# DeepMETv2/DeepMETv2

Hardware: AMD Instinct MI355X
Metric: events/sec (4.5k PF cands, k=16) (higher is better)
Workload: dtype f32

## Files before the change

### deepmetv2_amd/csrc/knn.hip

```cpp
#include <stdlib.h>

#include "common.h"
#include "nls_body.h"

namespace dmet {
namespace {

typedef float f2 __attribute__((ext_vector_type(2)));

constexpr int kTileC = 32;
constexpr int kQMax = 8;
constexpr int kMaxSplit = 8;
constexpr int kWavesPerGroup = 4;

__device__ __forceinline__ void wave_sync()
{
    __builtin_amdgcn_fence(__ATOMIC_RELEASE, "wavefront");
    __builtin_amdgcn_wave_barrier();
    __builtin_amdgcn_fence(__ATOMIC_ACQUIRE, "wavefront");
}

#define DMET_PKSUB_LO " op_sel:[0,0] op_sel_hi:[0,1] neg_lo:[0,1] neg_hi:[0,1]\n\t"
#define DMET_PKSUB_HI " op_sel:[1,0] op_sel_hi:[1,1] neg_lo:[0,1] neg_hi:[0,1]\n\t"
__device__ __forceinline__ void pk_dist_step4(f2 &accA, f2 &accB, f2 vxy, f2 vzw, f2 wxy, f2 wzw, f2 q0, f2 q1, f2 q2,
// ... 658 lines not shown
    const int64_t *ptr;
    int B;
    int64_t N;
    int k;
    float *nrm;
    uint8_t *rec;
    const KnnPlan *plan;
    const int32_t *order;
    const int32_t *pos_of;
    const int32_t *tile_ptr;
    float *psd;
    int32_t *psj;
    int32_t *nbr;
    float *dist;
    uint16_t *nbr16;
    int32_t *flags;
    int32_t *any;
    uint8_t *qflag;
    int32_t *qlist;
    const int32_t *xtile_ptr;
    int xtile_queries;
    int form2;
    float slack_scale;
    const float *rW, *rb;
    float *rP, *rQ;
    int r_sliced;
    int first_rider;
    int emit_coalesced;
    int no_rerank;
};

struct KnnSizeHint {
    int min_nodes = 0, max_nodes = 0;
};
thread_local KnnSizeHint g_size_hint;

struct KnnRider {
    const float *W = nullptr, *b = nullptr;
    float *P = nullptr, *Q = nullptr;
    int sliced = 0;
    bool done = false;
};
thread_local KnnRider g_rider;

struct KnnAffine {
    const float *raw = nullptr, *res = nullptr, *gamma = nullptr, *beta = nullptr, *mean = nullptr, *invstd = nullptr;
    bool done = false;
};
thread_local KnnAffine g_affine;
inline int rider_groups()
{
    static int cached = 0;
    if (cached == 0) {
        const char *e = getenv("DMET_KNN_RIDER_GROUPS");
        const int v = e ? atoi(e) : 0;
        cached = (v >= 1 && v <= 4096) ? v : 512;
    }
    return cached;
}

__device__ __forceinline__ void flag_query(const KnnFilterArgs &a, int q, int xtile)
{
    a.qflag[q] = 1;
    atomicAdd(a.flags + xtile, 1);
    const int slot = atomicAdd(a.any, 1);
    if (slot < a.N) a.qlist[slot] = q;
}

__device__ __forceinline__ unsigned bf16_rne_bits(float f)
{
    const unsigned u = __float_as_uint(f);
    return (u + 0x7fffu + ((u >> 16) & 1u)) >> 16;
}

constexpr int kRecFragBytes = 4 * kWave * 16;
constexpr int rec_bytes(int NH) { return kRecFragBytes * NH + 32 * 4; }
constexpr int kRecBytes = rec_bytes(1);
constexpr int kRecBytesMax = rec_bytes(2);

__device__ __forceinline__ int64_t rec_base_tile(const int64_t *__restrict__ ptr, int b) { return (ptr[b] >> 5) + b; }

constexpr int kRec16FragBytes = 2 * kWave * 16;
constexpr float kF16WideLimit = 16384.0f;

__device__ __forceinline__ bool f2_in_domain64(int64_t n) { return n >= kF2MinNodes && n <= kF2MaxNodes; }

template <int NH, bool AFFINE = false>
__global__ __launch_bounds__(256) void knn_prep_kernel(const float *__restrict__ x, const int64_t *__restrict__ ptr,
                                                        int B, int64_t N, float *__restrict__ nrm,
                                                        uint8_t *__restrict__ rec, int64_t nrec,
                                                        uint32_t *__restrict__ zero, size_t zero_bytes, KnnPlanOut o0,
                                                        KnnPlanOut o1, int form2, KnnAffine af = KnnAffine{})
{
    static_assert(!AFFINE || NH == 1, "the fused BatchNorm transform is built for 32 features");
    const int64_t t = (int64_t)blockIdx.x * blockDim.x + threadIdx.x;
    {
        const size_t words = zero_bytes >> 2, total = (size_t)gridDim.x * blockDim.x;
        for (size_t wd = (size_t)t; wd < words; wd += total) zero[wd] = 0u;
        if (t == 0)
            for (size_t bt = words << 2; bt < zero_bytes; ++bt) reinterpret_cast<uint8_t *>(zero)[bt] = 0;
    }
    if (blockIdx.x + 2 >= gridDim.x) {
        knn_plan_body(ptr, B, blockIdx.x + 2 == gridDim.x ? o0 : o1);
        return;
    }
    const int64_t tile = (int64_t)blockIdx.x * (blockDim.x >> 6) + __builtin_amdgcn_readfirstlane((int)(threadIdx.x >> 6));
    if (tile >= nrec) return;
    const int lane = (int)(t & 63), col = lane & 31, hh = lane >> 5;
    int lo = 0, hi = B;
    {
        const int ln = (int)(threadIdx.x & 63);
        while (hi - lo > 1) {
            const int span = hi - lo, step = (span + 63) >> 6;
            const int cand = lo + step * (ln + 1);
            const bool ok = cand < hi && rec_base_tile(ptr, cand) <= tile;
            const unsigned long long m = __ballot(ok);
            const int cnt = __popcll(m);
            const int nlo = lo + step * cnt;
            const int nhi = min(hi, lo + step * (cnt + 1));
            lo = __builtin_amdgcn_readfirstlane(nlo);
            hi = __builtin_amdgcn_readfirstlane(nhi);
        }
    }
    const int64_t ev_lo = ptr[lo], n = ptr[lo + 1] - ev_lo;
    const int64_t li0 = (tile - rec_base_tile(ptr, lo)) * 32;
    if (li0 >= n) return;
    const bool live = li0 + col < n;
    const int64_t r = ev_lo + (live ? li0 + col : 0);
    const bool rec16 = form2 != 0 && f2_in_domain64(n);
    float s = 0.0f;
    uint8_t *recp = rec + tile * rec_bytes(NH);
    float f[NH][16];
    if constexpr (NH == 1) {
        __shared__ __attribute__((aligned(16))) float prep_tile[4][32 * 36];
        float *T = prep_tile[threadIdx.x >> 6];
        const int fg = lane & 7;
        float4 mu4, sc4, be4;
        if constexpr (AFFINE) {
            mu4 = reinterpret_cast<const float4 *>(af.mean)[fg];
            const float4 is4 = reinterpret_cast<const float4 *>(af.invstd)[fg], ga4 = reinterpret_cast<const float4 *>(af.gamma)[fg];
            be4 = reinterpret_cast<const float4 *>(af.beta)[fg];
            sc4 = make_float4(ga4.x * is4.x, ga4.y * is4.y, ga4.z * is4.z, ga4.w * is4.w);
        }
#pragma unroll
        for (int jj = 0; jj < 4; ++jj) {
            const int rowj = 8 * jj + (lane >> 3);
            const bool livej = li0 + rowj < n;
            const int64_t rj = ev_lo + (livej ? li0 + rowj : 0);
            float4 v;
            if constexpr (AFFINE) {
                const float4 a = reinterpret_cast<const float4 *>(af.raw + rj * 32)[fg];
                v.x = (a.x - mu4.x) * sc4.x + be4.x; v.y = (a.y - mu4.y) * sc4.y + be4.y;
                v.z = (a.z - mu4.z) * sc4.z + be4.z; v.w = (a.w - mu4.w) * sc4.w + be4.w;
                if (af.res) {
                    const float4 q = reinterpret_cast<const float4 *>(af.res + rj * 32)[fg];
                    v.x += q.x; v.y += q.y; v.z += q.z; v.w += q.w;
                }
                if (livej) reinterpret_cast<float4 *>(const_cast<float *>(x) + rj * 32)[fg] = v;
            } else {
                v = reinterpret_cast<const float4 *>(x + rj * 32)[fg];
            }
            *reinterpret_cast<float4 *>(&T[rowj * 36 + 4 * fg]) = v;
        }
        asm volatile("s_waitcnt lgkmcnt(0)" ::: "memory");
        __builtin_amdgcn_wave_barrier();
#pragma unroll
        for (int kb = 0; kb < 2; ++kb) {
            const float4 v0 = *reinterpret_cast<const float4 *>(&T[col * 36 + 16 * kb + 8 * hh]);
            const float4 v1 = *reinterpret_cast<const float4 *>(&T[col * 36 + 16 * kb + 8 * hh + 4]);
            f[0][8 * kb + 0] = v0.x; f[0][8 * kb + 1] = v0.y; f[0][8 * kb + 2] = v0.z; f[0][8 * kb + 3] = v0.w;
            f[0][8 * kb + 4] = v1.x; f[0][8 * kb + 5] = v1.y; f[0][8 * kb + 6] = v1.z; f[0][8 * kb + 7] = v1.w;
        }
    } else {
#pragma unroll
        for (int half = 0; half < NH; ++half) {
#pragma unroll
            for (int kb = 0; kb < 2; ++kb) {
                const float4 *g = reinterpret_cast<const float4 *>(x + r * (32 * NH) + 32 * half + 16 * kb + 8 * hh);
                const float4 v0 = g[0], v1 = g[1];
                f[half][8 * kb + 0] = v0.x; f[half][8 * kb + 1] = v0.y; f[half][8 * kb + 2] = v0.z; f[half][8 * kb + 3] = v0.w;
                f[half][8 * kb + 4] = v1.x; f[half][8 * kb + 5] = v1.y; f[half][8 * kb + 6] = v1.z; f[half][8 * kb + 7] = v1.w;
            }
        }
    }
    bool wide = false;
#pragma unroll
    for (int half = 0; half < NH; ++half) {
#pragma unroll
        for (int u = 0; u < 16; ++u) {
            const float v = live ? f[half][u] : 0.0f;
            f[half][u] = v;
            s = __builtin_fmaf(v, v, s);
            wide = wide || !(__builtin_fabsf(v) < kF16WideLimit);
        }
    }
    s += __shfl_xor(s, 32, 64);
    if (rec16) {
        wide = wide || (__shfl_xor(wide ? 1 : 0, 32, 64) != 0);
#pragma unroll
        for (int half = 0; half < NH; ++half) {
            uint4 *dst = reinterpret_cast<uint4 *>(recp + half * kRec16FragBytes);
#pragma unroll
            for (int kb = 0; kb < 2; ++kb) {
                f16x8 hv;
#pragma unroll
                for (int u = 0; u < 8; ++u) hv[u] = wide ? (_Float16)0.0f : (_Float16)f[half][8 * kb + u];
                dst[kb * 64 + lane] = __builtin_bit_cast(uint4, hv);
            }
        }
        if (hh == 0) {
            reinterpret_cast<float *>(recp + kRec16FragBytes * NH)[col] =
                !live ? __builtin_inff() : (wide ? -__builtin_inff() : s);
            if (live) nrm[r] = s;
        }
        return;
    }
#pragma unroll
    for (int half = 0; half < NH; ++half) {
        unsigned h[16], m[16];
#pragma unroll
        for (int u = 0; u < 16; ++u) {
            const float v = f[half][u];
            h[u] = bf16_rne_bits(v);
            m[u] = bf16_rne_bits(v - __uint_as_float(h[u] << 16));
        }
        uint4 *dst = reinterpret_cast<uint4 *>(recp + half * kRecFragBytes);
#pragma unroll
        for (int kb = 0; kb < 2; ++kb) {
            dst[kb * 64 + lane] = make_uint4(h[8 * kb] | (h[8 * kb + 1] << 16), h[8 * kb + 2] | (h[8 * kb + 3] << 16),
                                             h[8 * kb + 4] | (h[8 * kb + 5] << 16), h[8 * kb + 6] | (h[8 * kb + 7] << 16));
            dst[(2 + kb) * 64 + lane] = make_uint4(m[8 * kb] | (m[8 * kb + 1] << 16), m[8 * kb + 2] | (m[8 * kb + 3] << 16),
                                                   m[8 * kb + 4] | (m[8 * kb + 5] << 16), m[8 * kb + 6] | (m[8 * kb + 7] << 16));
        }
    }
    if (!live) s = __builtin_inff();
    if (hh == 0) {
        reinterpret_cast<float *>(recp + kRecFragBytes * NH)[col] = s;
        if (live) nrm[r] = s;
    }
}

template <int NH = 1>
__device__ __forceinline__ f32x16 filter_block(const bf16x8 (&av)[4 * NH], const bf16x8 (&bv)[4 * NH], const f32x16 &cinit)
{
    f32x16 acc = cinit;
#pragma unroll
    for (int h = 0; h < NH; ++h) {
        acc = __builtin_amdgcn_mfma_f32_32x32x16_bf16(av[4 * h + 0], bv[4 * h + 0], acc, 0, 0, 0);
        acc = __builtin_amdgcn_mfma_f32_32x32x16_bf16(av[4 * h + 1], bv[4 * h + 1], acc, 0, 0, 0);
        acc = __builtin_amdgcn_mfma_f32_32x32x16_bf16(av[4 * h + 0], bv[4 * h + 2], acc, 0, 0, 0);
        acc = __builtin_amdgcn_mfma_f32_32x32x16_bf16(av[4 * h + 1], bv[4 * h + 3], acc, 0, 0, 0);
        acc = __builtin_amdgcn_mfma_f32_32x32x16_bf16(av[4 * h + 2], bv[4 * h + 0], acc, 0, 0, 0);
        acc = __builtin_amdgcn_mfma_f32_32x32x16_bf16(av[4 * h + 3], bv[4 * h + 1], acc, 0, 0, 0);
    }
    return acc;
}

template <int NH = 1>
__device__ __forceinline__ void filter_load(bf16x8 (&av)[4 * NH], f32x16 &cinit, const uint8_t *__restrict__ rec,
                                            int64_t tidx, int lane, int hh)
{
    const uint8_t *base = rec + tidx * rec_bytes(NH);
    const bf16x8 *g = reinterpret_cast<const bf16x8 *>(base);
#pragma unroll
    for (int m = 0; m < 4 * NH; ++m) av[m] = g[m * 64 + lane];
    const float4 *nr = reinterpret_cast<const float4 *>(base + kRecFragBytes * NH);
#pragma unroll
    for (int q = 0; q < 4; ++q) {
        const float4 v = nr[2 * q + hh];
        cinit[4 * q] = v.x; cinit[4 * q + 1] = v.y; cinit[4 * q + 2] = v.z; cinit[4 * q + 3] = v.w;
    }
}

template <int M>
struct FilterLane {
    float tk[M];
    float tau;
    int cnt;
    int kept;
    bool overflow;
};

constexpr int filter_list_len(int KP) { return KP + 4; }
constexpr int filter_queue_len(int M) { return M + 28; }

template <int QF>
struct FilterQueue {
    unsigned key[QF][kWave];
    unsigned short id[QF][kWave];
};

template <int M>
__device__ __forceinline__ void filter_drain(FilterLane<M> &L, FilterQueue<filter_queue_len(M)> &Q, int lane)
{
    constexpr int QF = filter_queue_len(M);
    int maxnew = L.cnt - L.kept;
#pragma unroll
// ... 263 lines not shown
                                (unsigned)local_id16(kj[p], ev_lo) | ((unsigned)local_id16(kj[p + 1], ev_lo) << 16);
                } else {
#pragma unroll
                    for (int p = 0; p < KP; ++p)
                        if (p < k) r16[p] = local_id16(kj[p], ev_lo);
                }
            }
            const float tau = L.tk[M - 1];
            const float nx = a.nrm[myq];
            const float an = __builtin_sqrtf(nx) * 1.000001f;
            const float rn = an + __builtin_sqrtf(fmaxf(kth, 0.0f)) * 1.00002f;
            const float slack = 2.0f * (4e-5f * an * rn + 1e-5f * rn * rn + 4e-6f * an * an) + 1e-30f;
            const bool full = tau < kKnnSentinel;
            if (L.overflow || !fits || (full && !(tau + nx - slack > kth))) {
                flag_query(a, myq, a.xtile_ptr[pos] + (myq - ev_lo) / a.xtile_queries);
            }
        }
        return;
    }
    if (a.no_rerank) {
        if (valid && sub == 0) flag_query(a, myq, a.xtile_ptr[pos] + (myq - ev_lo) / a.xtile_queries);
        return;
    }
    if (valid) {
        const int64_t slot = (int64_t)(tile - n_full) * kFQ + hh * 32 + col;
        float *ld = a.psd + (slot * nsub + sub) * MS;
        int32_t *lj = a.psj + (slot * nsub + sub) * MS;
        const float tfin = L.tk[M - 1];
        int out = 0;
        for (int pass = 0; pass < 2; ++pass)
            for (int s = 0; s < L.cnt; ++s) {
                const float key = __uint_as_float(Q.key[s][lane]);
                if ((pass == 0 ? key < tfin : key == tfin) && out < M) {
                    ld[out] = key;
                    lj[out] = ev_lo + (int32_t)Q.id[s][lane];
                    ++out;
                }
            }
        for (; out < M; ++out) { ld[out] = kKnnSentinel; lj[out] = -1; }
        ld[M] = L.tk[M - 1];
        lj[M] = (L.overflow || !fits) ? 1 : 0;
    }
}

template <int KP>
__global__ __launch_bounds__(kWave * kWavesPerGroup, 2) void knn_filter_kernel(const KnnFilterArgs a)
{
    __shared__ FilterQueue<filter_queue_len(filter_list_len(KP))> queue_all[kWavesPerGroup];
    const int wv = __builtin_amdgcn_readfirstlane(threadIdx.x >> 6), lane = threadIdx.x & 63;
    filter1_wave<KP>(a, queue_all[wv], (int)blockIdx.x, wv, lane);
}


#ifndef DMET_F2_DEFER
#define DMET_F2_DEFER 32
#endif
constexpr int kF2Defer = DMET_F2_DEFER;
#ifdef DMET_F2_LEAN
constexpr int kF2Slots = 26;
constexpr int kF2StageRows = 4;
constexpr int kF2WavesPerSimd = 3;
#else
constexpr int kF2Slots = 30;
constexpr int kF2StageRows = kWave;
constexpr int kF2WavesPerSimd = 2;
#endif
constexpr int kF2RowF = 16;
constexpr unsigned kF2TileBits = 11u, kF2TileMask = (1u << kF2TileBits) - 1u;

struct F2Wave {
    uint2 ent[kF2Slots][kWave];
    float rows[kF2StageRows][kF2RowF + 4];
};
#ifndef DMET_F2_LEAN
static_assert(sizeof(F2Wave) == 20480, "two workgroups of four wavefronts fill the CU's 160 KB exactly");
#else
static_assert(sizeof(F2Wave) * 12 <= 163840, "three workgroups of four wavefronts per CU");
#endif

template <int M>
struct F2Lane {
    float tk[M];
    float tau;
    int cnt;
    bool overflow;
};

template <int M>
__device__ __forceinline__ void f2_compact(F2Lane<M> &L, F2Wave &S, int lane, int limit)
{
    const float tauT = __uint_as_float(__float_as_uint(L.tau) & ~kF2TileMask);
    int maxcnt = L.cnt;
#pragma unroll
    for (int off = 32; off > 0; off >>= 1) maxcnt = max(maxcnt, __shfl_xor(maxcnt, off, 64));
    int out = 0;
    for (int s = 0; s < maxcnt; ++s) {
        if (s < L.cnt) {
            const uint2 e = S.ent[s][lane];
            if (!(__uint_as_float(e.y & ~kF2TileMask) > tauT)) { S.ent[out][lane] = e; ++out; }
        }
    }
    L.cnt = out;
    if (out > limit) {
        L.overflow = true;
        L.cnt = 0;
        L.tau = -__builtin_inff();
    }
}

template <int NH = 1>
struct F2Ops {
    f16x8 a[2 * NH];
    f32x16 c;
};

template <int NH = 1>
__device__ __forceinline__ f32x16 f2_block(const f16x8 (&av)[2 * NH], const f16x8 (&bv)[2 * NH], const f32x16 &cinit)
{
    f32x16 acc = cinit;
#pragma unroll
    for (int m = 0; m < 2 * NH; ++m) acc = __builtin_amdgcn_mfma_f32_32x32x16_f16(av[m], bv[m], acc, 0, 0, 0);
    return acc;
}

template <int NH = 1>
__device__ __forceinline__ void f2_load(F2Ops<NH> &o, const uint8_t *__restrict__ rec, int64_t tidx, int lane, int hh)
{
    const uint8_t *base = rec + tidx * rec_bytes(NH);
    const f16x8 *g = reinterpret_cast<const f16x8 *>(base);
#pragma unroll
    for (int m = 0; m < 2 * NH; ++m) o.a[m] = g[m * 64 + lane];
    const float4 *nr = reinterpret_cast<const float4 *>(base + kRec16FragBytes * NH);
#pragma unroll
    for (int q = 0; q < 4; ++q) {
        const float4 v = nr[2 * q + hh];
        o.c[4 * q] = v.x; o.c[4 * q + 1] = v.y; o.c[4 * q + 2] = v.z; o.c[4 * q + 3] = v.w;
    }
}

__device__ __forceinline__ float f2_slack(float an, float rn, float scale)
{
    return 2.0f * scale * (4e-5f * an * rn + 1e-5f * rn * rn + 4e-6f * an * an) + 1.96e-3f * an * rn + 6e-7f * (an + rn) +
           1e-30f;
}

constexpr int f2_list_len(int KP) { return KP <= 16 ? KP + 6 : KP + 4; }

__device__ __forceinline__ int f2_mask_row(int p) { return (p & 3) + 8 * ((p & 15) >> 2) + 4 * (p >> 4); }

template <int M, bool UPD, bool REC, bool INS, int NH = 1>
__device__ __forceinline__ void f2_tile(F2Lane<M> &L, F2Wave &S, const uint8_t *__restrict__ rec, int64_t rbase, int t,
                                        int t_hi, f32x16 &c0, f32x16 &c1, f32x16 &n0, f32x16 &n1, const F2Ops<NH> &use,
                                        F2Ops<NH> &ld, const f16x8 (&bq)[2][2 * NH], int lane, int hh, bool alive,
                                        float &carry)
{
#if defined(DMET_F2_ABL) && DMET_F2_ABL >= 2
    constexpr bool kRec = false;
#else
    constexpr bool kRec = REC;
#endif
#if defined(DMET_F2_ABL) && DMET_F2_ABL >= 3
    constexpr bool kUpd = false;
#else
    constexpr bool kUpd = UPD;
#endif
    if (kRec) {
        if (__any(L.cnt >= kF2Slots - 1)) f2_compact<M>(L, S, lane, kF2Slots - 3);
    }
#if defined(DMET_F2_SAMEREC)
    f2_load<NH>(ld, rec, rbase + (t & 1), lane, hh);
#else
    f2_load<NH>(ld, rec, rbase + min(t + 2, t_hi - 1), lane, hh);
#endif
    n0 = f2_block<NH>(use.a, bq[0], use.c);
    n1 = f2_block<NH>(use.a, bq[1], use.c);
    unsigned mask = 0u;
    if (kRec) {
        const auto tt = __builtin_amdgcn_permlane32_swap(__float_as_uint(L.tau), __float_as_uint(L.tau), false, false);
        const float t0 = __uint_as_float(tt[0]), t1 = __uint_as_float(tt[1]);
        unsigned ma = 0u, mb = 0u;
#pragma unroll
        for (int e = 0; e < 16; ++e) {
            ma = __builtin_amdgcn_alignbit(ma, __float_as_uint(c0[e] - t0), 31);
            mb = __builtin_amdgcn_alignbit(mb, __float_as_uint(c1[e] - t1), 31);
        }
        const auto mm = __builtin_amdgcn_permlane32_swap(ma, mb, false, false);
        mask = (mm[0] << 16) | mm[1];
    }
    float tmin = -__builtin_inff();
    if (kUpd) {
        float na = kKnnSentinel, nb = kKnnSentinel;
#pragma unroll
        for (int e = 0; e < 16; e += 2) {
            asm("v_min3_f32 %0, %0, %1, %2" : "+v"(na) : "v"(c0[e]), "v"(c0[e + 1]));
            asm("v_min3_f32 %0, %0, %1, %2" : "+v"(nb) : "v"(c1[e]), "v"(c1[e + 1]));
        }
        const auto nn = __builtin_amdgcn_permlane32_swap(__float_as_uint(na), __float_as_uint(nb), false, false);
        tmin = __uint_as_float(nn[0]);
        asm("v_min_f32 %0, %0, %1" : "+v"(tmin) : "v"(__uint_as_float(nn[1])));
    }
    if (kRec) {
        const unsigned packed = (__float_as_uint(tmin) & ~kF2TileMask) | (unsigned)t;
        S.ent[L.cnt][lane] = make_uint2(mask, packed);
        L.cnt += (mask != 0u) ? 1 : 0;
    }
    if (kUpd) {
        if (INS) {
            float v = tmin < -3.0e38f ? kKnnSentinel : tmin;
            asm("v_min_f32 %0, %0, %1" : "+v"(v) : "v"(carry));
            carry = kKnnSentinel;
#pragma unroll
            for (int p = M - 1; p >= 1; --p) L.tk[p] = __builtin_amdgcn_fmed3f(L.tk[p - 1], v, L.tk[p]);
            asm("v_min_f32 %0, %0, %1" : "+v"(L.tk[0]) : "v"(v));
            if (alive && !L.overflow) L.tau = L.tk[M - 1];
        } else {
            carry = tmin;
        }
    }
#ifdef DMET_F2_SCHED
#pragma unroll
    for (int g = 0; g < 12; ++g) {
        __builtin_amdgcn_sched_group_barrier(0x008, 1, 0);
        __builtin_amdgcn_sched_group_barrier(0x002, (kRec ? 11 : (kUpd ? 5 : 2)), 0);
    }
#endif
}

template <int M, bool UPD, bool REC, int NH = 1>
__device__ __forceinline__ void f2_sweep(F2Lane<M> &L, F2Wave &S, const uint8_t *__restrict__ rec, int64_t rbase,
                                         int t_lo, int t_hi, const f16x8 (&bq)[2][2 * NH], int lane, int hh, bool alive)
{
    if (t_lo >= t_hi) return;
    F2Ops<NH> A, B;
    f2_load<NH>(A, rec, rbase + t_lo, lane, hh);
    f32x16 c0 = f2_block<NH>(A.a, bq[0], A.c);
    f32x16 c1 = f2_block<NH>(A.a, bq[1], A.c);
    f32x16 n0, n1;
    f2_load<NH>(A, rec, rbase + min(t_lo + 1, t_hi - 1), lane, hh);
    float carry = kKnnSentinel;
    for (int t = t_lo; t < t_hi; t += 2) {
        f2_tile<M, UPD, REC, true, NH>(L, S, rec, rbase, t, t_hi, c0, c1, n0, n1, A, B, bq, lane, hh, alive, carry);
        if (t + 1 < t_hi)
            f2_tile<M, UPD, REC, true, NH>(L, S, rec, rbase, t + 1, t_hi, n0, n1, c0, c1, B, A, bq, lane, hh, alive, carry);
    }
}

__device__ __forceinline__ int filter_group(const KnnFilterArgs &a)
{
    const int full_groups = a.plan->n_full / kWavesPerGroup;
    return (int)blockIdx.x < full_groups ? xcd_swizzle((int)blockIdx.x, full_groups) : (int)blockIdx.x;
}

template <int KP, int NH = 1>
__device__ __forceinline__ void filter2_wave(const KnnFilterArgs &a, F2Wave &S, int *tickets, int group, int wv, int lane)
{
    constexpr int M = f2_list_len(KP);
    constexpr int D = 32 * NH;
    constexpr int MS = (M + 1 + 3) & ~3;
    const int col = lane & 31, hh = lane >> 5;
    const uint8_t *__restrict__ rec = a.rec;
    const int64_t *__restrict__ ptr = a.ptr;

    const int n_full = a.plan->n_full, split = a.plan->split, total = a.plan->total_tiles;
    const int item = group * kWavesPerGroup + wv;
    int tile = item, sub = 0, nsub = 1;
    if (item >= n_full) {
        const int r = item - n_full;
        tile = n_full + r / split;
        sub = r % split;
        nsub = split;
    }
    if (tile >= total) return;
    const int pos = find_tile_event(a.tile_ptr, a.B, tile);
    const int ev = a.order[pos];
    const int ev_lo = (int)ptr[ev], ev_hi = (int)ptr[ev + 1];
    const int q_first = ev_lo + (tile - a.tile_ptr[pos]) * kFQ;
    if (!f2_in_domain(ev_hi - ev_lo)) {
        if (NH != 1 && sub == 0) {
            const int q = q_first + lane;
            if (q < ev_hi) {
                flag_query(a, q, a.xtile_ptr[pos] + (q - ev_lo) / a.xtile_queries);
            }
        }
        return;
    }
    int clo = ev_lo, chi = ev_hi;
    bool idle_piece = false;
    if (nsub > 1) {
        if (ev_hi - ev_lo < kF2SplitMinNodes) {
            idle_piece = sub != 0;
        } else {
            const int chunk = (((chi - clo) + nsub - 1) / nsub + 31) & ~31;
            clo = min(chi, clo + sub * chunk);
            chi = min(chi, clo + chunk);
        }
    }
    const int64_t rbase = (ptr[ev] >> 5) + ev;
    const int64_t rlast = rbase + (ev_hi - ev_lo - 1) / 32;
    const int t_lo = (clo - ev_lo) / 32, t_hi = idle_piece ? t_lo : (chi - ev_lo + 31) / 32;

    const int myq = q_first + hh * 32 + col;
    const bool valid = myq < ev_hi;
    float t_fix = -__builtin_inff();
    bool act = valid;
    for (int attempt = 0;; ++attempt) {
    F2Lane<M> L;
#pragma unroll
    for (int p = 0; p < M; ++p) L.tk[p] = kKnnSentinel;
    L.tau = attempt == 0 ? -__builtin_inff() : t_fix;
    L.cnt = 0;
    L.overflow = false;
    {
        f16x8 bq[2][2 * NH];
#pragma unroll
        for (int b = 0; b < 2; ++b) {
            const int64_t qrec = min(rbase + (q_first - ev_lo) / 32 + b, rlast);
            const f16x8 *g = reinterpret_cast<const f16x8 *>(rec + qrec * rec_bytes(NH));
#pragma unroll
            for (int m = 0; m < 2 * NH; ++m) bq[b][m] = g[m * 64 + lane] * (_Float16)-2.0f;
        }
        if (attempt == 0) {
            const int t_def = min(t_hi, t_lo + kF2Defer);
            f2_sweep<M, true, false, NH>(L, S, rec, rbase, t_lo, t_def, bq, lane, hh, valid);
            f2_sweep<M, true, true, NH>(L, S, rec, rbase, t_def, t_hi, bq, lane, hh, valid);
            f2_sweep<M, false, true, NH>(L, S, rec, rbase, t_lo, t_def, bq, lane, hh, valid);
        } else {
            f2_sweep<M, false, true, NH>(L, S, rec, rbase, t_lo, t_hi, bq, lane, hh, valid);
        }
    }
    f2_compact<M>(L, S, lane, kF2Slots);
#if defined(DMET_F2_ABL) && DMET_F2_ABL >= 1
    return;
#endif

    const int64_t qrow_id = valid ? myq : ev_lo;
    float qrow[D];
    {
        const float4 *g = reinterpret_cast<const float4 *>(a.x + qrow_id * D);
#pragma unroll
        for (int c = 0; c < D / 4; ++c) {
            const float4 v = g[c];
            qrow[4 * c] = v.x; qrow[4 * c + 1] = v.y; qrow[4 * c + 2] = v.z; qrow[4 * c + 3] = v.w;
        }
    }
    unsigned long long kk[KP];
#pragma unroll
    for (int p = 0; p < KP; ++p) kk[p] = (unsigned long long)__float_as_uint(kKnnSentinel) << 32;
    const int nent = (act && !L.overflow) ? L.cnt : 0;
    int slot = 0;
    unsigned cmask = 0u;
    int ctile = 0;
    auto pop = [&]() __attribute__((always_inline)) -> int32_t {
        if (cmask == 0u && slot < nent) {
            const uint2 e = S.ent[slot][lane];
            cmask = e.x;
            ctile = (int)(e.y & kF2TileMask);
            ++slot;
        }
        int32_t j = -1;
        if (cmask != 0u) {
            const int r = __builtin_clz(cmask);
            cmask &= ~(0x80000000u >> r);
            j = ev_lo + ctile * 32 + f2_mask_row(r);
        }
        return j;
    };
    const float4 *x4 = reinterpret_cast<const float4 *>(a.x);
#ifdef DMET_RR_PRIO
    __builtin_amdgcn_s_setprio(DMET_RR_PRIO);
#endif
    if constexpr (NH != 1) {
        for (;;) {
            const int32_t j = pop();
            if (!__any(j >= 0)) break;
            const float4 *row = x4 + (int64_t)(j >= 0 ? j : ev_lo) * (D / 4);
            float4 v[D / 4];
#pragma unroll
            for (int c = 0; c < D / 4; ++c) v[c] = row[c];
            float dc = 0.0f;
#pragma unroll
            for (int c = 0; c < D / 4; ++c) {
                float df;
                df = v[c].x - qrow[4 * c + 0]; dc = __builtin_fmaf(df, df, dc);
                df = v[c].y - qrow[4 * c + 1]; dc = __builtin_fmaf(df, df, dc);
                df = v[c].z - qrow[4 * c + 2]; dc = __builtin_fmaf(df, df, dc);
                df = v[c].w - qrow[4 * c + 3]; dc = __builtin_fmaf(df, df, dc);
            }
            const unsigned long long nk =
                j >= 0 ? (((unsigned long long)__float_as_uint(dc) << 32) | (unsigned)j) : ~0ull;
            bool g[KP];
#pragma unroll
            for (int p = 0; p < KP; ++p) g[p] = kk[p] > nk;
// ... 153 lines not shown
                for (int t = 0; t < RP; ++t) {
                    const int pi = t * 64 + lane;
                    const uint4 v = *reinterpret_cast<const uint4 *>(stg + 4 * pi);
                    if ((on >> (pi / RP)) & 1ull) *reinterpret_cast<uint4 *>(a.nbr + blk + 4 * pi) = v;
                }
                wave_sync();
#pragma unroll
                for (int q = 0; q < RP; ++q)
                    *reinterpret_cast<uint4 *>(stg + lane * KP + 4 * q) =
                        make_uint4(__float_as_uint(kd[4 * q]), __float_as_uint(kd[4 * q + 1]), __float_as_uint(kd[4 * q + 2]),
                                   __float_as_uint(kd[4 * q + 3]));
                wave_sync();
#pragma unroll
                for (int t = 0; t < RP; ++t) {
                    const int pi = t * 64 + lane;
                    const uint4 v = *reinterpret_cast<const uint4 *>(stg + 4 * pi);
                    if ((on >> (pi / RP)) & 1ull) *reinterpret_cast<uint4 *>(a.dist + blk + 4 * pi) = v;
                }
                if (a.nbr16) {
                    if constexpr (KP % 8 == 0) {
                        constexpr int RH = KP / 8;
                        wave_sync();
#pragma unroll
                        for (int q = 0; q < RH; ++q) {
                            uint4 w;
                            w.x = (unsigned)local_id16(kj[8 * q], ev_lo) | ((unsigned)local_id16(kj[8 * q + 1], ev_lo) << 16);
                            w.y = (unsigned)local_id16(kj[8 * q + 2], ev_lo) | ((unsigned)local_id16(kj[8 * q + 3], ev_lo) << 16);
                            w.z = (unsigned)local_id16(kj[8 * q + 4], ev_lo) | ((unsigned)local_id16(kj[8 * q + 5], ev_lo) << 16);
                            w.w = (unsigned)local_id16(kj[8 * q + 6], ev_lo) | ((unsigned)local_id16(kj[8 * q + 7], ev_lo) << 16);
                            *reinterpret_cast<uint4 *>(stg + lane * (KP / 2) + 4 * q) = w;
                        }
                        wave_sync();
#pragma unroll
                        for (int t = 0; t < RH; ++t) {
                            const int pi = t * 64 + lane;
                            const uint4 v = *reinterpret_cast<const uint4 *>(stg + 4 * pi);
                            if ((on >> (pi / RH)) & 1ull)
                                *reinterpret_cast<uint4 *>(reinterpret_cast<unsigned *>(a.nbr16 + blk) + 4 * pi) = v;
                        }
                    } else if (rows_on) {
                        uint16_t *r16 = a.nbr16 + (int64_t)myq * k;
#pragma unroll
                        for (int p = 0; p + 1 < KP; p += 2)
                            reinterpret_cast<unsigned *>(r16)[p >> 1] =
                                (unsigned)local_id16(kj[p], ev_lo) | ((unsigned)local_id16(kj[p + 1], ev_lo) << 16);
                    }
                }
                wave_sync();
                return kth;
            }
        }
        if (!rows_on) return kth;
#pragma unroll
        for (int p = 0; p < KP; ++p) {
            if (p < k) {
                a.nbr[(int64_t)myq * k + p] = kj[p];
                a.dist[(int64_t)myq * k + p] = kd[p];
            }
        }
        if (a.nbr16) {
            uint16_t *r16 = a.nbr16 + (int64_t)myq * k;
            if ((k & 1) == 0) {
#pragma unroll
                for (int p = 0; p + 1 < KP; p += 2)
                    if (p < k)
                        reinterpret_cast<unsigned *>(r16)[p >> 1] =
                            (unsigned)local_id16(kj[p], ev_lo) | ((unsigned)local_id16(kj[p + 1], ev_lo) << 16);
            } else {
#pragma unroll
                for (int p = 0; p < KP; ++p)
                    if (p < k) r16[p] = local_id16(kj[p], ev_lo);
            }
        }
        return kth;
    };
    if (nsub == 1) {
        bool retry = false;
        const float kth = emit(act, true);
        if (act) {
            const float nx = a.nrm[myq];
            const float an = __builtin_sqrtf(nx) * 1.000001f;
            const float rn = an + __builtin_sqrtf(fmaxf(kth, 0.0f)) * 1.00002f;
            const float slack = f2_slack(an, rn, NH == 1 ? 1.0f : 1.5f);
            const bool full = tau < kKnnSentinel;
            const bool wideq = !(nx < kF16WideLimit * kF16WideLimit);
            const bool fail = L.overflow || wideq || (full && !(kth >= 0.0f && tau + nx - slack > kth));
            float ts = kth - nx + slack;
            ts += (__builtin_fabsf(ts) + nx + slack) * 4.8e-7f + 1e-30f;
            retry = fail && attempt == 0 && !L.overflow && !wideq && kth >= 0.0f && ts + nx - slack > kth &&
                    ts < kKnnSentinel;
            if (fail && !retry) {
                flag_query(a, myq, a.xtile_ptr[pos] + (myq - ev_lo) / a.xtile_queries);
#ifdef DMET_KNN_WHY
                a.qflag[myq] = (uint8_t)(1 | (L.overflow ? 2 : 0) | (wideq ? 4 : 0) | (kth < 0.0f ? 8 : 0) | (attempt ? 16 : 0) |
                                         (!(ts < kKnnSentinel) ? 32 : 0) | (!(ts + nx - slack > kth) ? 64 : 0));
                a.dist[(int64_t)myq * k + 0] = tau; a.dist[(int64_t)myq * k + 1] = kth; a.dist[(int64_t)myq * k + 2] = slack; a.dist[(int64_t)myq * k + 3] = (float)L.cnt;
#endif
            }
            t_fix = retry ? ts : -__builtin_inff();
        }
        if (!__any(retry)) return;
        act = retry;
        continue;
    }
    static_assert(kFilterMaxSplit == 2 && kWavesPerGroup % 2 == 0, "pairs of sub-sweeps share a workgroup");
    const int64_t fslot = (int64_t)(tile - n_full) * kFQ + hh * 32 + col;
    if (valid) {
        float *ld = a.psd + (fslot * nsub + sub) * MS;
        int32_t *lj = a.psj + (fslot * nsub + sub) * MS;
#pragma unroll
        for (int p = 0; p < KP; ++p) { ld[p] = kd[p]; lj[p] = kj[p]; }
        ld[M] = tau;
        lj[M] = L.overflow ? 1 : 0;
    }
    __builtin_amdgcn_fence(__ATOMIC_RELEASE, "workgroup");
    int arrived = 0;
    if (lane == 0) arrived = atomicAdd(&tickets[wv >> 1], 1);
    arrived = __builtin_amdgcn_readfirstlane(arrived);
    if (arrived == 0) return;
    __builtin_amdgcn_fence(__ATOMIC_ACQUIRE, "workgroup");
    float tau_o = kKnnSentinel;
    int of_o = 0;
    if (valid) {
        const float *ld = a.psd + (fslot * nsub + (sub ^ 1)) * MS;
        const int32_t *lj = a.psj + (fslot * nsub + (sub ^ 1)) * MS;
        tau_o = ld[M];
        of_o = lj[M];
#pragma unroll
        for (int p = 0; p < KP; ++p) {
            const float od = ld[p];
            const int32_t oj = lj[p];
            const unsigned long long nk = oj >= 0 ? (((unsigned long long)__float_as_uint(od) << 32) | (unsigned)oj) : ~0ull;
            bool g[KP];
#pragma unroll
            for (int q = 0; q < KP; ++q) g[q] = kk[q] > nk;
#pragma unroll
            for (int q = KP - 1; q >= 1; --q) kk[q] = g[q - 1] ? kk[q - 1] : (g[q] ? nk : kk[q]);
            kk[0] = g[0] ? nk : kk[0];
        }
#pragma unroll
        for (int p = 0; p < KP; ++p) {
            kd[p] = __uint_as_float((unsigned)(kk[p] >> 32));
            kj[p] = kd[p] == kKnnSentinel ? -1 : (int32_t)(unsigned)kk[p];
        }
        const float kth = emit(true, false);
        const float nx = a.nrm[myq];
        const float an = __builtin_sqrtf(nx) * 1.000001f;
        const float rn = an + __builtin_sqrtf(fmaxf(kth, 0.0f)) * 1.00002f;
        const float slack = f2_slack(an, rn, NH == 1 ? 1.0f : 1.5f);
        const bool wideq = !(nx < kF16WideLimit * kF16WideLimit);
        const bool fail_a = tau < kKnnSentinel && !(kth >= 0.0f && tau + nx - slack > kth);
        const bool fail_b = tau_o < kKnnSentinel && !(kth >= 0.0f && tau_o + nx - slack > kth);
        if (L.overflow || of_o != 0 || wideq || fail_a || fail_b)
            flag_query(a, myq, a.xtile_ptr[pos] + (myq - ev_lo) / a.xtile_queries);
    }
    return;
    }
}

template <int KP, int NH = 1>
__global__ __launch_bounds__(kWave * kWavesPerGroup, kF2WavesPerSimd) void knn_filter12_kernel(const KnnFilterArgs a)
{
    union WaveLds {
        F2Wave f2;
#ifndef DMET_F2_LEAN
        FilterQueue<filter_queue_len(filter_list_len(KP))> f1;
#endif
    };
    __shared__ WaveLds sh_all[kWavesPerGroup];
    if constexpr (NH == 1) {
        if (a.rP != nullptr && (int)blockIdx.x >= a.first_rider) {
            static_assert(sizeof(WaveLds) >= sizeof(float) * kNlsLdsFloats, "a wavefront's LDS holds the transposition tiles");
            const int rwv = __builtin_amdgcn_readfirstlane(threadIdx.x >> 6);
            const int64_t wave = (int64_t)((int)blockIdx.x - a.first_rider) * kWavesPerGroup + rwv;
            const int64_t nwaves = (int64_t)((int)gridDim.x - a.first_rider) * kWavesPerGroup;
            float *tp = reinterpret_cast<float *>(&sh_all[rwv]);
            if (a.r_sliced == 2)
                node_linear_split_bf16_wave<32, 32>(a.x, a.N, a.rW, a.rb, a.rP, reinterpret_cast<unsigned short *>(a.rQ), wave,
                                                    nwaves, threadIdx.x & 63);
            else if (a.r_sliced == 1) node_linear_split_wave<32, 32, true>(a.x, a.N, a.rW, a.rb, a.rP, a.rQ, tp, wave, nwaves, threadIdx.x & 63);
            else node_linear_split_wave<32, 32, false>(a.x, a.N, a.rW, a.rb, a.rP, a.rQ, tp, wave, nwaves, threadIdx.x & 63);
            return;
        }
    }
    static_assert(sizeof(WaveLds) == sizeof(F2Wave), "the union is sized by the second form");
#ifndef DMET_F2_LEAN
    static_assert(sizeof(FilterQueue<filter_queue_len(filter_list_len(KP))>) <= sizeof(F2Wave) - 8, "ticket bytes are free");
#endif
    static_assert(kWavesPerGroup / 2 <= 2, "two ticket words");
    int *tickets = reinterpret_cast<int *>(&sh_all[0].f2.rows[kF2StageRows - 1][kF2RowF + 2]);
    const int wv = __builtin_amdgcn_readfirstlane(threadIdx.x >> 6), lane = threadIdx.x & 63;
    if (threadIdx.x < kWavesPerGroup / 2) tickets[threadIdx.x] = 0;
    __syncthreads();
    const int group = filter_group(a);
    filter2_wave<KP, NH>(a, sh_all[wv].f2, tickets, group, wv, lane);
#ifndef DMET_F2_LEAN
    if constexpr (NH == 1) filter1_wave<KP>(a, sh_all[wv].f1, group, wv, lane);
#endif
}

template <int KP>
__global__ __launch_bounds__(256) void knn_rerank_kernel(const KnnFilterArgs a)
{
    constexpr int M = filter_list_len(KP);
    constexpr int MS = (M + 1 + 3) & ~3;
    constexpr int QPW = kWave / M;
    constexpr int QPB = 4 * QPW;
    constexpr int EMAX = kFilterMaxSplit * M;
    __shared__ float sc[QPB][EMAX];
    __shared__ int32_t sj[QPB][EMAX];
    __shared__ float skth[QPB];
    __shared__ int sfail[QPB];
    __shared__ float qbuf[QPB][32];
    constexpr int PARTS = (kFQ + QPB - 1) / QPB;
    const int wv = __builtin_amdgcn_readfirstlane(threadIdx.x >> 6), lane = threadIdx.x & 63;
    const int qw = lane / M, l = lane - qw * M;
    const int slot = wv * QPW + min(qw, QPW - 1);
    const int bid = blockIdx.x;
    if (a.form2 && a.plan->form1_events == 0) return;
    const int n_full = a.plan->n_full, split = a.plan->split;
    const int ft = n_full + bid / PARTS, part = bid % PARTS;
    if (ft >= a.plan->total_tiles) return;
    const int pos = find_tile_event(a.tile_ptr, a.B, ft);
    const int ev = a.order[pos];
    const int64_t ev_lo = a.ptr[ev], ev_hi = a.ptr[ev + 1];
    if (a.form2 && f2_in_domain((int)(ev_hi - ev_lo))) return;
    const int qoff = part * QPB + wv * QPW + qw;
    const int64_t q = ev_lo + (int64_t)(ft - a.tile_ptr[pos]) * kFQ + qoff;
    const bool active = qw < QPW && qoff < kFQ && q < ev_hi;
    const int64_t qq = active ? q : ev_lo;
    const int nsub = split;
    const int64_t fslot = (int64_t)(ft - n_full) * kFQ + (active ? qoff : 0);
    const float *bd = a.psd + fslot * nsub * MS;
    const int32_t *bj = a.psj + fslot * nsub * MS;
    const int E = nsub * M;
// ... 812 lines not shown
```

Baseline: 45890.

## Fold norm and threshold subtraction into an extra MFMA for the f16 KNN filter

For the 32-feature f16 filter path, the candidate norm is split into four f16 limbs stored in the record, and the running threshold tau is encoded as two f16 values. A leading MFMA then adds norm minus tau directly into the accumulator, so the per-element subtraction of tau before sign-bit mask extraction disappears. A conservative key lower bound and certification margins are added to keep the approximate tau exact-safe. The sweep is also reworked to triple-buffer records with a prefetch lead of three and to update the tau encoding only every other tile, trading an extra MFMA and more registers for fewer VALU ops.

```diff
diff --git a/deepmetv2_amd/csrc/knn.hip b/deepmetv2_amd/csrc/knn.hip
--- a/deepmetv2_amd/csrc/knn.hip
+++ b/deepmetv2_amd/csrc/knn.hip
@@ -764,6 +764,13 @@
 
 constexpr int kRec16FragBytes = 2 * kWave * 16;
 constexpr float kF16WideLimit = 16384.0f;
+static_assert(kRec16FragBytes + kWave * 16 <= rec_bytes(1) && 2 * kRec16FragBytes + kWave * 16 <= rec_bytes(2),
+              "the fold fragment fits the record");
+constexpr float kF2NormP[4] = {0x1p15f, 0x1p5f, 0x1p-6f, 0x1p-17f};
+constexpr float kF2NormInvP[4] = {0x1p-15f, 0x1p-5f, 0x1p6f, 0x1p17f};
+constexpr float kF2NormMax = 65504.0f * 0x1p15f;
+constexpr float kF2TauC[2] = {0x1p14f, 0x1p-15f};
+constexpr float kF2TauRepMax = 65504.0f * 0x1p14f;
 
 __device__ __forceinline__ bool f2_in_domain64(int64_t n) { return n >= kF2MinNodes && n <= kF2MaxNodes; }
 
@@ -890,11 +897,34 @@
                 dst[kb * 64 + lane] = __builtin_bit_cast(uint4, hv);
             }
         }
+        if constexpr (NH != 1) {
+            if (hh == 0) {
+                reinterpret_cast<float *>(recp + kRec16FragBytes * NH)[col] =
+                    !live ? __builtin_inff() : (wide ? -__builtin_inff() : s);
+                if (live) nrm[r] = s;
+            }
+            return;
+        }
+        f16x8 fv = {};
         if (hh == 0) {
-            reinterpret_cast<float *>(recp + kRec16FragBytes * NH)[col] =
-                !live ? __builtin_inff() : (wide ? -__builtin_inff() : s);
+            const float sn = !live ? __builtin_inff() : ((wide || !(s < kF2NormMax)) ? -__builtin_inff() : s);
+            if (sn == sn && __builtin_fabsf(sn) < __builtin_inff()) {
+                float rr = sn;
+#pragma unroll
+                for (int i = 0; i < 4; ++i) {
+                    const _Float16 h = (_Float16)(rr * kF2NormInvP[i]);
+                    fv[4 + i] = h;
+                    rr -= (float)h * kF2NormP[i];
+                }
+            } else {
+                fv[4] = (_Float16)sn;
+            }
             if (live) nrm[r] = s;
-        }
+        } else {
+            fv[0] = (_Float16)kF2TauC[0];
+            fv[1] = (_Float16)kF2TauC[1];
+        }
+        reinterpret_cast<uint4 *>(recp + kRec16FragBytes * NH)[lane] = __builtin_bit_cast(uint4, fv);
         return;
     }
 #pragma unroll
@@ -1324,6 +1354,8 @@
 struct F2Lane {
     float tk[M];
     float tau;
+    unsigned tq;
+    float rep;
     int cnt;
     bool overflow;
 };
@@ -1350,18 +1382,34 @@
     }
 }
 
+__device__ __forceinline__ f16x8 f2_fold(unsigned tq)
+{
+    const f16x8 pc = {(_Float16)0.0f, (_Float16)0.0f, (_Float16)0.0f, (_Float16)0.0f, (_Float16)kF2NormP[0],
+                      (_Float16)kF2NormP[1], (_Float16)kF2NormP[2], (_Float16)kF2NormP[3]};
+    uint4 u = __builtin_bit_cast(uint4, pc);
+    u.x = tq;
+    return __builtin_bit_cast(f16x8, u);
+}
+
 template <int NH = 1>
 struct F2Ops {
     f16x8 a[2 * NH];
+    f16x8 f;
+};
+template <>
+struct F2Ops<2> {
+    f16x8 a[4];
     f32x16 c;
 };
 
 template <int NH = 1>
-__device__ __forceinline__ f32x16 f2_block(const f16x8 (&av)[2 * NH], const f16x8 (&bv)[2 * NH], const f32x16 &cinit)
-{
-    f32x16 acc = cinit;
-#pragma unroll
-    for (int m = 0; m < 2 * NH; ++m) acc = __builtin_amdgcn_mfma_f32_32x32x16_f16(av[m], bv[m], acc, 0, 0, 0);
+__device__ __forceinline__ f32x16 f2_block(const F2Ops<NH> &o, const f16x8 (&bv)[2 * NH], unsigned tq)
+{
+    f32x16 acc;
+    if constexpr (NH == 1) acc = __builtin_amdgcn_mfma_f32_32x32x16_f16(o.f, f2_fold(tq), f32x16{}, 0, 0, 0);
+    else acc = o.c;
+#pragma unroll
+    for (int m = 0; m < 2 * NH; ++m) acc = __builtin_amdgcn_mfma_f32_32x32x16_f16(o.a[m], bv[m], acc, 0, 0, 0);
     return acc;
 }
 
@@ -1372,29 +1420,61 @@
     const f16x8 *g = reinterpret_cast<const f16x8 *>(base);
 #pragma unroll
     for (int m = 0; m < 2 * NH; ++m) o.a[m] = g[m * 64 + lane];
-    const float4 *nr = reinterpret_cast<const float4 *>(base + kRec16FragBytes * NH);
-#pragma unroll
-    for (int q = 0; q < 4; ++q) {
-        const float4 v = nr[2 * q + hh];
-        o.c[4 * q] = v.x; o.c[4 * q + 1] = v.y; o.c[4 * q + 2] = v.z; o.c[4 * q + 3] = v.w;
-    }
-}
+    if constexpr (NH == 1) {
+        o.f = g[2 * NH * 64 + lane];
+    } else {
+        const float4 *nr = reinterpret_cast<const float4 *>(base + kRec16FragBytes * NH);
+#pragma unroll
+        for (int q = 0; q < 4; ++q) {
+            const float4 v = nr[2 * q + hh];
+            o.c[4 * q] = v.x; o.c[4 * q + 1] = v.y; o.c[4 * q + 2] = v.z; o.c[4 * q + 3] = v.w;
+        }
+    }
+}
+
+__device__ __forceinline__ unsigned f2_tau16(float tau, float &rep)
+{
+    const float x = __builtin_amdgcn_fmed3f(-tau * (1.0f / kF2TauC[0]), -65504.0f, 65504.0f);
+    float v = __builtin_amdgcn_fmed3f(__builtin_fmaf(__builtin_fabsf(x), -0x1p-9f, x), -65504.0f, 65504.0f);
+    const float y0 = (float)__builtin_amdgcn_cvt_pkrtz(v, v)[0];
+    const float w = __builtin_fmaf(-y0, kF2TauC[0] / kF2TauC[1], x * (kF2TauC[0] / kF2TauC[1]));
+    v = fminf(__builtin_fmaf(__builtin_fabsf(w), -0x1p-9f, w - 0x1p-24f), 65504.0f);
+    const auto y = __builtin_amdgcn_cvt_pkrtz(y0, v);
+    rep = -__builtin_fmaf(y0, kF2TauC[0], (float)y[1] * kF2TauC[1]);
+    return __builtin_bit_cast(unsigned, y);
+}
+
+__device__ __forceinline__ float f2_key_lower(float cmin, float rep)
+{
+    const float s = cmin + rep;
+    return __builtin_fmaf(__builtin_fabsf(s), -0x1p-22f, __builtin_fmaf(__builtin_fabsf(rep), -0x1p-17f, s));
+}
+
+template <int NH = 1>
+__device__ __forceinline__ float f2_cert_T(float tau)
+{
+    if constexpr (NH != 1) return tau;
+    const float T = fminf(tau, kF2TauRepMax);
+    return __builtin_fmaf(__builtin_fabsf(T), -0x1p-16f, T) - 1e-16f;
+}
+template <int NH = 1>
+__device__ __forceinline__ bool f2_full(float tau) { return NH == 1 || tau < kKnnSentinel; }
 
 __device__ __forceinline__ float f2_slack(float an, float rn, float scale)
 {
     return 2.0f * scale * (4e-5f * an * rn + 1e-5f * rn * rn + 4e-6f * an * an) + 1.96e-3f * an * rn + 6e-7f * (an + rn) +
-           1e-30f;
+           6e-14f * rn * rn + 1e-12f;
 }
 
 constexpr int f2_list_len(int KP) { return KP <= 16 ? KP + 6 : KP + 4; }
 
 __device__ __forceinline__ int f2_mask_row(int p) { return (p & 3) + 8 * ((p & 15) >> 2) + 4 * (p >> 4); }
 
-template <int M, bool UPD, bool REC, bool INS, int NH = 1>
+template <int M, bool UPD, bool REC, bool INS, int NH = 1, bool CONV = true, int LEAD = 2>
 __device__ __forceinline__ void f2_tile(F2Lane<M> &L, F2Wave &S, const uint8_t *__restrict__ rec, int64_t rbase, int t,
-                                        int t_hi, f32x16 &c0, f32x16 &c1, f32x16 &n0, f32x16 &n1, const F2Ops<NH> &use,
-                                        F2Ops<NH> &ld, const f16x8 (&bq)[2][2 * NH], int lane, int hh, bool alive,
-                                        float &carry)
+                                        int t_hi, f32x16 &c0, f32x16 &c1, f32x16 &n0, f32x16 &n1, float &rc, float &rn,
+                                        const F2Ops<NH> &use, F2Ops<NH> &ld, const f16x8 (&bq)[2][2 * NH], int lane,
+                                        int hh, bool alive, float &carry)
 {
 #if defined(DMET_F2_ABL) && DMET_F2_ABL >= 2
     constexpr bool kRec = false;
@@ -1412,19 +1492,35 @@
 #if defined(DMET_F2_SAMEREC)
     f2_load<NH>(ld, rec, rbase + (t & 1), lane, hh);
 #else
-    f2_load<NH>(ld, rec, rbase + min(t + 2, t_hi - 1), lane, hh);
-#endif
-    n0 = f2_block<NH>(use.a, bq[0], use.c);
-    n1 = f2_block<NH>(use.a, bq[1], use.c);
+    f2_load<NH>(ld, rec, rbase + min(t + LEAD, t_hi - 1), lane, hh);
+#endif
+    {
+        unsigned q0 = 0u, q1 = 0u;
+        if (NH == 1 && kRec) {
+            const auto tt = __builtin_amdgcn_permlane32_swap(L.tq, L.tq, false, false);
+            q0 = tt[0]; q1 = tt[1];
+        }
+        n0 = f2_block<NH>(use, bq[0], q0);
+        n1 = f2_block<NH>(use, bq[1], q1);
+        rn = L.rep;
+    }
     unsigned mask = 0u;
     if (kRec) {
-        const auto tt = __builtin_amdgcn_permlane32_swap(__float_as_uint(L.tau), __float_as_uint(L.tau), false, false);
-        const float t0 = __uint_as_float(tt[0]), t1 = __uint_as_float(tt[1]);
         unsigned ma = 0u, mb = 0u;
-#pragma unroll
-        for (int e = 0; e < 16; ++e) {
-            ma = __builtin_amdgcn_alignbit(ma, __float_as_uint(c0[e] - t0), 31);
-            mb = __builtin_amdgcn_alignbit(mb, __float_as_uint(c1[e] - t1), 31);
+        if constexpr (NH == 1) {
+#pragma unroll
+            for (int e = 0; e < 16; ++e) {
+                ma = __builtin_amdgcn_alignbit(ma, __float_as_uint(c0[e]), 31);
+                mb = __builtin_amdgcn_alignbit(mb, __float_as_uint(c1[e]), 31);
+            }
+        } else {
+            const auto tt = __builtin_amdgcn_permlane32_swap(__float_as_uint(L.tau), __float_as_uint(L.tau), false, false);
+            const float t0 = __uint_as_float(tt[0]), t1 = __uint_as_float(tt[1]);
+#pragma unroll
+            for (int e = 0; e < 16; ++e) {
+                ma = __builtin_amdgcn_alignbit(ma, __float_as_uint(c0[e] - t0), 31);
+                mb = __builtin_amdgcn_alignbit(mb, __float_as_uint(c1[e] - t1), 31);
+            }
         }
         const auto mm = __builtin_amdgcn_permlane32_swap(ma, mb, false, false);
         mask = (mm[0] << 16) | mm[1];
@@ -1440,6 +1536,7 @@
         const auto nn = __builtin_amdgcn_permlane32_swap(__float_as_uint(na), __float_as_uint(nb), false, false);
         tmin = __uint_as_float(nn[0]);
         asm("v_min_f32 %0, %0, %1" : "+v"(tmin) : "v"(__uint_as_float(nn[1])));
+        if (NH == 1 && kRec) tmin = f2_key_lower(tmin, rc);
     }
     if (kRec) {
         const unsigned packed = (__float_as_uint(tmin) & ~kF2TileMask) | (unsigned)t;
@@ -1455,6 +1552,7 @@
             for (int p = M - 1; p >= 1; --p) L.tk[p] = __builtin_amdgcn_fmed3f(L.tk[p - 1], v, L.tk[p]);
             asm("v_min_f32 %0, %0, %1" : "+v"(L.tk[0]) : "v"(v));
             if (alive && !L.overflow) L.tau = L.tk[M - 1];
+            if (NH == 1 && kRec && CONV) L.tq = f2_tau16(L.tau, L.rep);
         } else {
             carry = tmin;
         }
@@ -1475,15 +1573,48 @@
     if (t_lo >= t_hi) return;
     F2Ops<NH> A, B;
     f2_load<NH>(A, rec, rbase + t_lo, lane, hh);
-    f32x16 c0 = f2_block<NH>(A.a, bq[0], A.c);
-    f32x16 c1 = f2_block<NH>(A.a, bq[1], A.c);
+    unsigned q0 = 0u, q1 = 0u;
+    if (NH == 1 && REC) {
+        L.tq = f2_tau16(L.tau, L.rep);
+        const auto tt = __builtin_amdgcn_permlane32_swap(L.tq, L.tq, false, false);
+        q0 = tt[0]; q1 = tt[1];
+    }
+    float rc = L.rep, rn;
+    f32x16 c0 = f2_block<NH>(A, bq[0], q0);
+    f32x16 c1 = f2_block<NH>(A, bq[1], q1);
     f32x16 n0, n1;
     f2_load<NH>(A, rec, rbase + min(t_lo + 1, t_hi - 1), lane, hh);
     float carry = kKnnSentinel;
+    if constexpr (NH == 1 && UPD && REC) {
+        F2Ops<NH> C;
+        f2_load<NH>(B, rec, rbase + min(t_lo + 2, t_hi - 1), lane, hh);
+        for (int t = t_lo; t < t_hi; t += 6) {
+            f2_tile<M, UPD, REC, true, NH, false, 3>(L, S, rec, rbase, t, t_hi, c0, c1, n0, n1, rc, rn, A, C, bq, lane, hh,
+                                                     alive, carry);
+            if (t + 1 >= t_hi) break;
+            f2_tile<M, UPD, REC, true, NH, true, 3>(L, S, rec, rbase, t + 1, t_hi, n0, n1, c0, c1, rn, rc, B, A, bq, lane,
+                                                    hh, alive, carry);
+            if (t + 2 >= t_hi) break;
+            f2_tile<M, UPD, REC, true, NH, false, 3>(L, S, rec, rbase, t + 2, t_hi, c0, c1, n0, n1, rc, rn, C, B, bq, lane,
+                                                     hh, alive, carry);
+            if (t + 3 >= t_hi) break;
+            f2_tile<M, UPD, REC, true, NH, true, 3>(L, S, rec, rbase, t + 3, t_hi, n0, n1, c0, c1, rn, rc, A, C, bq, lane,
+                                                    hh, alive, carry);
+            if (t + 4 >= t_hi) break;
+            f2_tile<M, UPD, REC, true, NH, false, 3>(L, S, rec, rbase, t + 4, t_hi, c0, c1, n0, n1, rc, rn, B, A, bq, lane,
+                                                     hh, alive, carry);
+            if (t + 5 >= t_hi) break;
+            f2_tile<M, UPD, REC, true, NH, true, 3>(L, S, rec, rbase, t + 5, t_hi, n0, n1, c0, c1, rn, rc, C, B, bq, lane,
+                                                    hh, alive, carry);
+        }
+        return;
+    }
     for (int t = t_lo; t < t_hi; t += 2) {
-        f2_tile<M, UPD, REC, true, NH>(L, S, rec, rbase, t, t_hi, c0, c1, n0, n1, A, B, bq, lane, hh, alive, carry);
+        f2_tile<M, UPD, REC, true, NH, false>(L, S, rec, rbase, t, t_hi, c0, c1, n0, n1, rc, rn, A, B, bq, lane, hh, alive,
+                                              carry);
         if (t + 1 < t_hi)
-            f2_tile<M, UPD, REC, true, NH>(L, S, rec, rbase, t + 1, t_hi, n0, n1, c0, c1, B, A, bq, lane, hh, alive, carry);
+            f2_tile<M, UPD, REC, true, NH, true>(L, S, rec, rbase, t + 1, t_hi, n0, n1, c0, c1, rn, rc, B, A, bq, lane, hh,
+                                                 alive, carry);
     }
 }
 
@@ -1550,6 +1681,8 @@
 #pragma unroll
     for (int p = 0; p < M; ++p) L.tk[p] = kKnnSentinel;
     L.tau = attempt == 0 ? -__builtin_inff() : t_fix;
+    L.tq = 0u;
+    L.rep = 0.0f;
     L.cnt = 0;
     L.overflow = false;
     {
@@ -1869,18 +2002,17 @@
             const float an = __builtin_sqrtf(nx) * 1.000001f;
             const float rn = an + __builtin_sqrtf(fmaxf(kth, 0.0f)) * 1.00002f;
             const float slack = f2_slack(an, rn, NH == 1 ? 1.0f : 1.5f);
-            const bool full = tau < kKnnSentinel;
             const bool wideq = !(nx < kF16WideLimit * kF16WideLimit);
-            const bool fail = L.overflow || wideq || (full && !(kth >= 0.0f && tau + nx - slack > kth));
+            const bool fail = L.overflow || wideq || (f2_full<NH>(tau) && !(kth >= 0.0f && f2_cert_T<NH>(tau) + nx - slack > kth));
             float ts = kth - nx + slack;
-            ts += (__builtin_fabsf(ts) + nx + slack) * 4.8e-7f + 1e-30f;
-            retry = fail && attempt == 0 && !L.overflow && !wideq && kth >= 0.0f && ts + nx - slack > kth &&
+            ts += __builtin_fabsf(ts) * ((NH == 1 ? 0x1p-15f : 0.0f) + 4.8e-7f) + (nx + slack) * 4.8e-7f + (NH == 1 ? 2e-16f : 1e-30f);
+            retry = fail && attempt == 0 && !L.overflow && !wideq && kth >= 0.0f && f2_cert_T<NH>(ts) + nx - slack > kth &&
                     ts < kKnnSentinel;
             if (fail && !retry) {
                 flag_query(a, myq, a.xtile_ptr[pos] + (myq - ev_lo) / a.xtile_queries);
 #ifdef DMET_KNN_WHY
                 a.qflag[myq] = (uint8_t)(1 | (L.overflow ? 2 : 0) | (wideq ? 4 : 0) | (kth < 0.0f ? 8 : 0) | (attempt ? 16 : 0) |
-                                         (!(ts < kKnnSentinel) ? 32 : 0) | (!(ts + nx - slack > kth) ? 64 : 0));
+                                         (!(ts < kKnnSentinel) ? 32 : 0) | (!(f2_cert_T<NH>(ts) + nx - slack > kth) ? 64 : 0));
                 a.dist[(int64_t)myq * k + 0] = tau; a.dist[(int64_t)myq * k + 1] = kth; a.dist[(int64_t)myq * k + 2] = slack; a.dist[(int64_t)myq * k + 3] = (float)L.cnt;
 #endif
             }
@@ -1936,8 +2068,8 @@
         const float rn = an + __builtin_sqrtf(fmaxf(kth, 0.0f)) * 1.00002f;
         const float slack = f2_slack(an, rn, NH == 1 ? 1.0f : 1.5f);
         const bool wideq = !(nx < kF16WideLimit * kF16WideLimit);
-        const bool fail_a = tau < kKnnSentinel && !(kth >= 0.0f && tau + nx - slack > kth);
-        const bool fail_b = tau_o < kKnnSentinel && !(kth >= 0.0f && tau_o + nx - slack > kth);
+        const bool fail_a = f2_full<NH>(tau) && !(kth >= 0.0f && f2_cert_T<NH>(tau) + nx - slack > kth);
+        const bool fail_b = f2_full<NH>(tau_o) && !(kth >= 0.0f && f2_cert_T<NH>(tau_o) + nx - slack > kth);
         if (L.overflow || of_o != 0 || wideq || fail_a || fail_b)
             flag_query(a, myq, a.xtile_ptr[pos] + (myq - ev_lo) / a.xtile_queries);
     }
```

Measured after the change: 47580, median of 6. +3.7%, better.
